# software-mansion/smelter

Measured on NVIDIA H100. Metric: 4K composited frames/sec (16-input grid) per GPU, higher is better.
Workload: dtype f32 math on u8 planes (f16 resampler scratch)

## Files before the change

include/smelter_b200.h:

```cpp
#ifndef SMELTER_B200_H
#define SMELTER_B200_H

#include <stddef.h>
#include <stdint.h>

#ifdef __cplusplus
extern "C" {
#endif

typedef struct smr_renderer smr_renderer;

typedef enum {
    SMR_OK = 0,
    SMR_ERR_INVALID_ARGUMENT = 1,
    SMR_ERR_CUDA = 2,
    SMR_ERR_OUTPUT_NOT_REGISTERED = 3,
    SMR_ERR_SCENE = 4,
    SMR_ERR_UNSUPPORTED = 5,
    SMR_ERR_OUT_OF_MEMORY = 6,
    SMR_ERR_BUFFER_TOO_SMALL = 7
} smr_status;

typedef enum { SMR_MODE_GPU_OPTIMIZED = 0, SMR_MODE_CPU_OPTIMIZED = 1 } smr_rendering_mode;

// ... 254 lines not shown
    uint32_t n_glyphs;
    const smr_atlas *mask_atlas, *color_atlas;
    int32_t color_mode;
} smr_text;

smr_status smr_debug_partition(const int32_t *dst_w, const int32_t *dst_h, uint32_t n_jobs, uint32_t max_blocks,
                               int32_t *pieces, uint32_t pieces_cap, uint32_t *n_pieces, int32_t *begin,
                               uint32_t begin_cap, uint32_t *n_blocks);

smr_status smr_debug_weights(float scale, float offset, uint32_t n_out, float *weights, size_t cap, uint32_t *taps, float *inv,
                             int32_t *first);
smr_status smr_debug_sincos(const float *x, uint32_t n, float *s, float *c);

smr_status smr_debug_tile_plan(const int32_t *boxes, uint32_t n_layers, uint32_t width, uint32_t height, int32_t sorted,
                               int32_t *owner_layer, uint32_t owner_cap, uint32_t *tiles, uint32_t tiles_cap, uint32_t *n_tiles);

typedef enum {
    SMR_FUSED_LDG = 0,
    SMR_FUSED_TMA_INT = 1,
    SMR_FUSED_TMA_ANY = 2
} smr_fused_kernel;
typedef struct {
    int32_t kernel;
    int32_t ratio;
    int32_t window;
    int32_t box;
    int32_t src_class;
    int32_t full_range;
    int32_t v_same;
    int32_t strip_cols;
// ... 103 lines not shown
```

smelter_b200/_ffi.py:

```python
import ctypes as C
import os

_HERE = os.path.dirname(os.path.abspath(__file__))
LIB_PATH = os.environ.get("SMR_LIB_PATH") or os.path.join(_HERE, "libsmelter_b200.so")

SMR_OK = 0
STATUS_NAMES = {0: "SMR_OK", 1: "SMR_ERR_INVALID_ARGUMENT", 2: "SMR_ERR_CUDA", 3: "SMR_ERR_OUTPUT_NOT_REGISTERED",
                4: "SMR_ERR_SCENE", 5: "SMR_ERR_UNSUPPORTED", 6: "SMR_ERR_OUT_OF_MEMORY", 7: "SMR_ERR_BUFFER_TOO_SMALL"}

MODE_GPU_OPTIMIZED, MODE_CPU_OPTIMIZED = 0, 1
COMPONENT_INPUT_STREAM, COMPONENT_VIEW, COMPONENT_TILES, COMPONENT_RESCALER = 0, 1, 2, 3
COMPONENT_SHADER, COMPONENT_WEB_VIEW, COMPONENT_IMAGE, COMPONENT_TEXT = 4, 5, 6, 7
FRAME_PLANAR_YUV420, FRAME_PLANAR_YUVJ420, FRAME_NV12, FRAME_BGRA, FRAME_ARGB, FRAME_RGBA8 = 0, 1, 2, 3, 4, 5
FRAME_PLANAR_YUV422, FRAME_PLANAR_YUV444, FRAME_UYVY422, FRAME_YUYV422 = 6, 7, 8, 9
MEM_HOST, MEM_DEVICE = 0, 1
WEB_CHROMIUM_EMBEDDING, WEB_NATIVE_OVER_CONTENT, WEB_NATIVE_UNDER_CONTENT = 0, 1, 2
OUT_PLANAR_YUV420, OUT_PLANAR_YUV422, OUT_PLANAR_YUV444, OUT_RGBA8, OUT_NV12 = 0, 1, 2, 3, 4
MAX_MASKS = 20


class Options(C.Structure):
    _fields_ = [("cuda_device", C.c_int32), ("rendering_mode", C.c_int32), ("max_layouts_count", C.c_uint32),
                ("stream_fallback_timeout_ns", C.c_uint64), ("framerate_num", C.c_uint32), ("framerate_den", C.c_uint32)]

# ... 175 lines not shown
                ("tex_pitch", C.c_int32 * 3), ("tex_align", C.c_int32 * 3), ("width", C.c_int32), ("height", C.c_int32),
                ("out_format", C.c_int32)]


KERNEL_CLASSES = ["convert", "weights", "resample_box", "resample_first", "resample_last", "composite", "output",
                  "fill", "resample_fused", "image", "web", "shader"]


class KernelTimes(C.Structure):
    _fields_ = [("total_ms", C.c_double * len(KERNEL_CLASSES)), ("launches", C.c_uint64 * len(KERNEL_CLASSES))]


EXPORTS = [
    "smr_create", "smr_destroy", "smr_register_input", "smr_unregister_input", "smr_register_image", "smr_unregister_image",
    "smr_register_web_renderer", "smr_unregister_web_renderer", "smr_web_set_frame", "smr_web_set_child_rects", "smr_register_shader", "smr_unregister_shader", "smr_register_wgsl_shader", "smr_update_scene",
    "smr_unregister_output", "smr_set_layouts", "smr_render", "smr_render_begin", "smr_render_end", "smr_preprocess_frame", "smr_premultiply_rgba8", "smr_render_text", "smr_debug_partition", "smr_debug_tile_plan", "smr_debug_weights", "smr_debug_sincos", "smr_debug_fused_jobs", "smr_debug_resample_stages", "smr_debug_composite_layers", "smr_debug_interior", "smr_output_plane_sizes",
    "smr_component_default", "smr_debug_layouts", "smr_debug_node_layouts", "smr_debug_image_nodes", "smr_debug_set_inputs", "smr_get_stats", "smr_set_profiling", "smr_get_kernel_times",
    "smr_comm_get_unique_id", "smr_comm_init", "smr_comm_broadcast_inputs", "smr_comm_exchange_inputs", "smr_comm_pull_inputs", "smr_peer_pool_alloc", "smr_peer_pool_open", "smr_peer_pool_close", "smr_peer_pool_free", "smr_comm_destroy", "smr_host_register", "smr_host_unregister", "smr_cuda_stream", "smr_last_error",
    "smr_version",
]

_lib = None


def lib():
    global _lib
    if _lib is not None:
        return _lib
    if not os.path.exists(LIB_PATH):
        raise ImportError(
            f"{LIB_PATH} is missing: build it with `python -m smelter_b200.build` "
# ... 20 lines not shown
        f.argtypes = [vp, C.c_uint64, C.POINTER(InputFrame), C.c_uint32, C.POINTER(OutputFrame), C.c_uint32]
    L.smr_render_end.argtypes = [vp]
    L.smr_preprocess_frame.argtypes = [vp, C.POINTER(InputFrame), C.c_uint32, C.c_uint32, C.c_void_p, C.c_uint32, C.c_int32]
    L.smr_preprocess_frame.restype = C.c_int32
    L.smr_premultiply_rgba8.argtypes = [vp, C.POINTER(InputFrame), C.c_void_p, C.c_uint32, C.c_int32]
    L.smr_premultiply_rgba8.restype = C.c_int32
    L.smr_render_text.argtypes = [vp, C.c_uint32, C.c_uint32, Rgba, C.c_void_p, C.c_uint32, C.POINTER(Atlas), C.POINTER(Atlas),
                                  C.c_int32, C.c_void_p, C.c_uint32, C.c_int32]
    L.smr_render_text.restype = C.c_int32
    L.smr_debug_partition.argtypes = [C.POINTER(C.c_int32), C.POINTER(C.c_int32), C.c_uint32, C.c_uint32, C.POINTER(C.c_int32),
                                      C.c_uint32, C.POINTER(C.c_uint32), C.POINTER(C.c_int32), C.c_uint32, C.POINTER(C.c_uint32)]
    L.smr_debug_partition.restype = C.c_int32
    L.smr_debug_tile_plan.argtypes = [C.POINTER(C.c_int32), C.c_uint32, C.c_uint32, C.c_uint32, C.c_int32, C.POINTER(C.c_int32), C.c_uint32,
                                      C.POINTER(C.c_uint32), C.c_uint32, C.POINTER(C.c_uint32)]
    L.smr_debug_tile_plan.restype = C.c_int32
    L.smr_debug_weights.argtypes = [C.c_float, C.c_float, C.c_uint32, C.c_void_p, C.c_size_t, C.POINTER(C.c_uint32), C.c_void_p,
                                    C.c_void_p]
    L.smr_debug_weights.restype = C.c_int32
    L.smr_debug_sincos.argtypes = [C.c_void_p, C.c_uint32, C.c_void_p, C.c_void_p]
    L.smr_debug_sincos.restype = C.c_int32
    L.smr_debug_fused_jobs.argtypes = [vp, C.POINTER(FusedJobInfo), C.c_uint32, C.POINTER(C.c_uint32)]
    L.smr_debug_fused_jobs.restype = C.c_int32
    L.smr_debug_resample_stages.argtypes = [vp, C.POINTER(ResampleStageInfo), C.c_uint32, C.POINTER(C.c_uint32),
                                            C.POINTER(C.c_int32), C.c_uint32, C.POINTER(C.c_uint32)]
    L.smr_debug_resample_stages.restype = C.c_int32
    L.smr_debug_composite_layers.argtypes = [vp, C.POINTER(CompositeLayerInfo), C.c_uint32, C.POINTER(C.c_uint32)]
    L.smr_debug_composite_layers.restype = C.c_int32
    L.smr_debug_interior.argtypes = [C.POINTER(RenderLayout), C.c_uint32, C.c_uint32, C.POINTER(C.c_int32 * 12), C.c_void_p]
    L.smr_debug_interior.restype = C.c_int32
    L.smr_output_plane_sizes.argtypes = [C.c_uint32, C.c_uint32, C.c_int32, C.POINTER(C.c_size_t * 3)]
# ... 35 lines not shown
```

smelter_b200/csrc/kernels.cu:

```cuda
#include <cuda_fp16.h>
#include <cuda_runtime.h>

#include <cstdio>
#include <cstdlib>
#include <atomic>
#include <cstring>

#include "kernels.h"
#include "interior.h"
#include "int_weights.h"

namespace smr {
namespace dev {

#include "ptx_helpers.cuh"

#define ENC_KEY0 ((127 - 13) << 5)
#define ENC_KEYS ((13 << 5) + 1)
__device__ unsigned char c_enc0[420];

#include "node_sample.cuh"

static thread_local char g_err[256] = {0};
const char *last_launch_error() { return g_err; }
// ... 880 lines not shown
#define PARAM_LAYERS kCompositeParamLayers
#define MAX_LUT 4
struct CompositeParams {
    CompositeJob job;
    LayerDev layers[PARAM_LAYERS];
};

template <bool PARAM>
__device__ __forceinline__ void composite_body(const CompositeJob &J, const LayerDev *__restrict__ LAYERS) {
    __shared__ Tables T;
    __shared__ unsigned short s_list[MAX_TILE_LAYERS];
    __shared__ int s_count;
    __shared__ LayerDev s_layers[PARAM ? 1 : SM_LAYERS];
    static_assert(CB_X * CT_W == kDirectTileW && CB_Y * CT_H * CT_ITERS == kDirectTileH, "direct tiles are the block tiles");
    int tile_x = blockIdx.x, tile_y = blockIdx.y;
    if (J.tile_list != nullptr) {
        if ((int)blockIdx.x >= J.n_tiles || blockIdx.y != 0) return;
        const uint32_t t = __ldg(J.tile_list + blockIdx.x);
        tile_x = (int)(t & 0xffffu); tile_y = (int)(t >> 16);
    } else if (J.direct_map != nullptr && __ldg(J.direct_map + tile_y * J.map_w + tile_x)) return;
    load_tables(T);
    const int tile_x0 = tile_x * (CB_X * CT_W), tile_y0 = tile_y * (CB_Y * CT_H * CT_ITERS);
    const int tile_x1 = min(tile_x0 + CB_X * CT_W, J.width), tile_y1 = min(tile_y0 + CB_Y * CT_H * CT_ITERS, J.height);
    {
        __shared__ int s_wc[CB_Y];
        const int tid = threadIdx.y * CB_X + threadIdx.x;
        int base_count = 0;
        for (int base = 0; base < J.n_layers; base += CB_X * CB_Y) {
            const int i = base + tid;
            bool hit = false;
            if (i < J.n_layers) {
                int4 bb;
                if (PARAM) bb = make_int4(LAYERS[i].px0, LAYERS[i].px1, LAYERS[i].py0, LAYERS[i].py1);
                else bb = __ldg(reinterpret_cast<const int4 *>(&LAYERS[i].px0));
                hit = bb.x < tile_x1 && bb.y > tile_x0 && bb.z < tile_y1 && bb.w > tile_y0;
            }
            const unsigned m = __ballot_sync(0xffffffffu, hit);
            if (threadIdx.x == 0) s_wc[threadIdx.y] = __popc(m);
            __syncthreads();
// ... 11 lines not shown
    }
    __syncthreads();
    if (!PARAM) {
        const int nsm = min(s_count, SM_LAYERS);
        const int words = (int)(sizeof(LayerDev) / 4);
        const int tid = threadIdx.y * CB_X + threadIdx.x;
        for (int i = tid; i < nsm * words; i += CB_X * CB_Y) {
            int l = i / words, w = i - l * words;
            reinterpret_cast<unsigned int *>(&s_layers[l])[w] =
                __ldg(reinterpret_cast<const unsigned int *>(&LAYERS[s_list[l]]) + w);
        }
    }
    __syncthreads();

    __shared__ uchar4 s_lut[MAX_LUT][CB_X * CB_Y];
    __shared__ uchar4 s_px[CB_Y][CB_X * CT_W * CT_H];
    __shared__ unsigned char s_items[CB_Y][CB_X * CT_W * CT_H];
    static_assert(CB_X == 32 && CB_X * CT_W * CT_H <= 256, "one warp per tile row, items fit a byte");
    static_assert(CB_X * CB_Y == 256, "one table entry per thread");
    {
        const int tid = threadIdx.y * CB_X + threadIdx.x;
        int nl = 0;
        for (int li = 0; li < s_count && nl < MAX_LUT; li++) {
            const LayerDev &L = PARAM ? LAYERS[s_list[li]] : (li < SM_LAYERS ? s_layers[li] : LAYERS[s_list[li]]);
            if (L.fast & FAST_LUT) {
                s_lut[nl][tid] = blend(T, J.mode, make_uchar4(tid, tid, tid, tid),
                                       make_float4(L.color[0], L.color[1], L.color[2], L.color[3]));
                nl++;
            }
        }
        if (nl) __syncthreads();
    }

// ... 176 lines not shown
                            px[j][i] = blend(T, J.mode, px[j][i], make_float4(lut[t.x], lut[t.y], lut[t.z], T.u8n[t.w]));
                        }
                    }
                break;
            }
            general = true;
        } while (0);
        unsigned need = 0;
        if (general) {
#pragma unroll 1
            for (int k = 0; k < CT_W * CT_H; k++) {
                const int X = x0 + (k & (CT_W - 1)), Y = y0 + k / CT_W;
                if (X < J.width && Y < J.height && quad_covers(L, X, Y)) need |= 1u << k;
            }
        }
        if (__ballot_sync(0xffffffffu, need != 0) == 0) continue;
        const int lane = threadIdx.x;
        const int cnt = __popc(need);
        int incl = cnt;
#pragma unroll
        for (int d = 1; d < 32; d <<= 1) {
            const int t = __shfl_up_sync(0xffffffffu, incl, d);
            if (lane >= d) incl += t;
        }
        const int total = __shfl_sync(0xffffffffu, incl, 31);
        if (total > 5 * 32) {
            for (int k = 0; k < CT_W * CT_H; k++) {
                if (!((need >> k) & 1u)) continue;
                const int i = k & (CT_W - 1), j = k / CT_W;
                uchar4 cur = j == 0 ? (i == 0 ? px[0][0] : i == 1 ? px[0][1] : i == 2 ? px[0][2] : px[0][3])
                                    : (i == 0 ? px[1][0] : i == 1 ? px[1][1] : i == 2 ? px[1][2] : px[1][3]);
                uchar4 res = shade_blend(T, J, L, x0 + i, y0 + j, cur);
#pragma unroll
                for (int jj = 0; jj < CT_H; jj++)
#pragma unroll
                    for (int ii = 0; ii < CT_W; ii++)
                        if (jj == j && ii == i) px[jj][ii] = res;
            }
            continue;
        }
        unsigned char *items = s_items[threadIdx.y];
        uchar4 *spx = s_px[threadIdx.y];
        if (need) {
            int o = incl - cnt;
#pragma unroll
            for (int k = 0; k < CT_W * CT_H; k++) {
                spx[lane * (CT_W * CT_H) + k] = px[k / CT_W][k & (CT_W - 1)];
                if ((need >> k) & 1u) items[o++] = (unsigned char)(lane * (CT_W * CT_H) + k);
            }
        }
        __syncwarp();
        for (int base = 0; base < total; base += 32) {
            const int idx = base + lane;
            if (idx < total) {
                const int item = items[idx], k = item & (CT_W * CT_H - 1);
                const int X = tile_x0 + (item / (CT_W * CT_H)) * CT_W + (k & (CT_W - 1)), Y = y0 + k / CT_W;
                spx[item] = shade_blend(T, J, L, X, Y, spx[item]);
            }
        }
        __syncwarp();
        if (need) {
#pragma unroll
            for (int k = 0; k < CT_W * CT_H; k++) px[k / CT_W][k & (CT_W - 1)] = spx[lane * (CT_W * CT_H) + k];
        }
    }

    if (x0 >= J.width || y0 >= J.height) continue;
    if (J.out_format < 0 || J.out_format == 3) {
        const bool vec16 = (((uintptr_t)J.out0 | (uintptr_t)J.out_pitch0) & 15) == 0;
#pragma unroll
        for (int j = 0; j < CT_H; j++) {
            int Y = y0 + j;
            if (Y >= J.height) break;
            uchar4 *row = reinterpret_cast<uchar4 *>(J.out0 + (size_t)Y * J.out_pitch0);
            if (x0 + CT_W <= J.width && vec16) {
                uint4 v;
                v.x = *reinterpret_cast<unsigned int *>(&px[j][0]);
                v.y = *reinterpret_cast<unsigned int *>(&px[j][1]);
// ... 335 lines not shown
```

smelter_b200/csrc/kernels.h:

```cpp
#pragma once

#include <cstddef>
#include <cstdint>

namespace smr {
namespace dev {

enum TexKind : int32_t {
    TEX_NONE = 0,
    TEX_RGBA8 = 1,
    TEX_YUV420 = 2,
    TEX_NV12 = 3,
    TEX_F16 = 4,
    TEX_BGRA = 5,
    TEX_ARGB = 6,
    TEX_YUV422 = 7,
    TEX_YUV444 = 8,
    TEX_UYVY = 9,
    TEX_YUYV = 10,
};
inline
#ifdef __CUDACC__
__host__ __device__
#endif
// ... 42 lines not shown

struct CompositeJob {
    int32_t width, height;
    int32_t mode;
    int32_t n_layers;
    const LayerDev *layers;
    const uint32_t *tile_list;
    const MaskDev *masks;
    const Tex *textures;
    int32_t out_format;
    uint8_t *out0, *out1, *out2;
    int32_t out_pitch0, out_pitch1, out_pitch2;
    const uint8_t *direct_map;
    int32_t map_w;
    int32_t n_tiles;
};
constexpr int kDirectTileW = 128, kDirectTileH = 16;
constexpr int kCompositeParamLayers = 96;

constexpr uint64_t kMaxBoxTexels = 1ull << 24;

struct ResampleJob {
    Tex src;
    int32_t axis;
    int32_t perp_offset;
    int32_t taps;
    int32_t dst_w, dst_h;
    int32_t dst_f16;
    uint8_t *dst;
    int32_t dst_pitch;
// ... 149 lines not shown
```

smelter_b200/csrc/node_sample.cuh:

```cuda

__device__ float c_u8n[256];
__device__ float c_dec[256];
__device__ float c_thr[256];
__device__ float c_yl[256];
#define ENC1_KEY0 ((127 - 13) << 8)
#define ENC1_KEYS ((13 << 8) + 1)
__device__ unsigned char c_enc1[ENC1_KEYS + 3];

struct Tables {
    float u8n[256];
    float dec[256];
    float thr[256];
    float yl[256];
};

__device__ __forceinline__ void load_tables(Tables &t) {
    for (int i = threadIdx.y * blockDim.x + threadIdx.x; i < 256; i += blockDim.x * blockDim.y) {
        t.u8n[i] = c_u8n[i];
        t.dec[i] = c_dec[i];
        t.thr[i] = c_thr[i];
        t.yl[i] = c_yl[i];
    }
    __syncthreads();
}

__device__ __forceinline__ float clamp01(float x) { return __saturatef(x); }

__device__ __forceinline__ int unorm8(float x) { return __float2int_rn(clamp01(x) * 255.0f); }

__device__ __forceinline__ int srgb_encode(const Tables &t, float lin) {
    const float x = clamp01(lin);
    const int k = max((__float_as_int(x) >> 15) - ENC1_KEY0, 0);
    const int e = __ldg(c_enc1 + k);
    return e + (x >= t.thr[e] ? 1 : 0);
}

struct LinTap {
// ... 285 lines not shown
```

smelter_b200/csrc/renderer.cpp:

```cpp
#include <cuda.h>
#include <cuda_runtime.h>
#include <dlfcn.h>

#include <algorithm>
#include <array>
#include <cmath>
#include <cstdio>
#include <cstring>
#include <deque>
#include <map>
#include <memory>
#include <mutex>
#include <string>
#include <tuple>
#include <vector>

#include "../../include/smelter_b200.h"
#include "interior.h"
#include "kernels.h"
#include "scene.h"
#include "wgsl.h"

namespace smr {

// ... 395 lines not shown
    struct Output {
        OutputNode node;
        std::vector<std::unique_ptr<TextNode>> texts;
        std::vector<std::unique_ptr<ImageNode>> images;
        std::vector<std::unique_ptr<WebNode>> webs;
        std::vector<std::unique_ptr<ShaderNode>> shaders;
        std::deque<Input> nested;
        uint64_t nodes_planned = 0;
        int32_t format = 0;
        Resolution res;
        DevBuf planes[kTicksInFlight][3];
        uint64_t tile_key = 0;
        bool tile_key_valid = false;
        std::vector<int> tile_owner_layer;
        std::vector<uint32_t> tile_list;
    };
    struct WeightKey {
        uint32_t scale_bits, offset_bits;
        int32_t n_out;
        bool operator<(const WeightKey &o) const {
            return std::tie(scale_bits, offset_bits, n_out) < std::tie(o.scale_bits, o.offset_bits, o.n_out);
        }
    };
    struct WeightEntry {
        float *weights = nullptr, *inv = nullptr;
        int32_t *first = nullptr;
        int taps = 0;
        uint64_t last_used = 0;
    };

// ... 85 lines not shown
    };
    struct StageRec {
        dev::ResampleJob job;
        int src_tex;
        size_t src_off, dst_off;
    };
    struct OutputRec { dev::OutputJob job; int src_tex; };
    struct CompositeRec {
        dev::CompositeJob job; size_t layers_off, masks_off;
        size_t out_frame_off = SIZE_MAX;
        size_t direct_off = SIZE_MAX;
        std::vector<int> direct_owner;
        bool use_list = false;
        std::vector<uint32_t> list;
        size_t list_off = SIZE_MAX;
    };
    struct PendingCopy { void *dst; size_t dpitch; const void *src; size_t spitch; size_t width, height; };
    struct Fill { uint8_t *p[3]; int pitch[3]; int w, h, fmt; uint8_t yuv[3]; };
    struct TickPlan {
        std::vector<TexRec> tex;
        std::vector<StageRec> stages[3];
        std::vector<FusedRec> fused;
        std::vector<CUtensorMap> tmaps;
        std::vector<dev::WeightJob> weight_jobs;
        std::vector<std::pair<int, size_t>> convert_jobs;
        std::vector<CompositeRec> composites;
        std::vector<OutputRec> outputs;
        std::vector<Fill> fills;
        std::vector<PendingCopy> d2h;
        std::vector<TextNode *> texts;
// ... 17 lines not shown
    smr_status make_image_node(const ImageParams &p, std::unique_ptr<ImageNode> &out);
    smr_status make_web_node(const WebParams &p, std::unique_ptr<WebNode> &out);
    void plan_web_node(Output &o, WebNode &n);
    smr_status make_shader_node(const ShaderParams &p, std::unique_ptr<ShaderNode> &out);
    void plan_shader_node(Output &o, ShaderNode &n, uint64_t pts);
    std::vector<std::pair<void *, cudaEvent_t>> retired_shaders_;
    void reap_shaders(bool all);
    cudaEvent_t web_ev_ = nullptr;
    cudaMemPool_t web_pool_ = nullptr;
    smr_status alloc_on_stream(size_t bytes, std::shared_ptr<void> &buf);
    Output &install_output(const char *output_id, OutputNode &&node, int32_t fmt, uint32_t w, uint32_t h);
    void plan_node_textures(Output &o, uint64_t pts);
    CompositeRec composite_rec(int W, int H, const std::vector<dev::LayerDev> &layers, const std::vector<dev::MaskDev> &masks);
    int composite_texture(CompositeRec pc);
    void plan_tiles(Output &o, CompositeRec &pc, const std::vector<dev::LayerDev> &layers, int W, int H);
    std::vector<WeightKey> new_weight_keys_;
    void rollback_weights();
    struct TmapKey {
        uintptr_t p; int pitch, w, h, kind;
        bool operator<(const TmapKey &o) const { return std::tie(p, pitch, w, h, kind) < std::tie(o.p, o.pitch, o.w, o.h, o.kind); }
    };
    std::map<TmapKey, CUtensorMap> tmap_cache_;
    std::map<std::tuple<uint32_t, uint32_t, int32_t, int32_t>, uint8_t *> lane_perms_;
    const uint8_t *lane_perm(float scale, float offset, int n_out, int cols);
    bool plane_tmap(const uint8_t *p, int pitch, int w, int h, int kind, CUtensorMap *out);
    bool direct_k11_ = true;

    std::vector<uint8_t> param_host_;
    size_t param_used_ = 0;
    PinnedBuf param_pinned_[kTicksInFlight];
    DevBuf param_dev_[kTicksInFlight];
    size_t frame_used_ = 0;
    DevBuf frame_dev_;
    std::map<WeightKey, WeightEntry> weights_;
    cudaStream_t copy_stream_ = nullptr, copy_stream2_ = nullptr;
    cudaStream_t d2h_stream_ = nullptr;
    cudaEvent_t kernels_done_[kTicksInFlight] = {};
    cudaEvent_t h2d_done2_[kTicksInFlight] = {};
    int upload_rr_ = 0;
    cudaEvent_t h2d_done_[kTicksInFlight] = {}, tick_done_[kTicksInFlight] = {};
    cudaStream_t comm_stream_ = nullptr;
// ... 73 lines not shown
    }
}

static double eotf_f64(double c) { return c <= 0.04045 ? c / 12.92 : std::pow((c + 0.055) / 1.055, 2.4); }
static const std::array<float, 255> kSrgbEncodeThr = [] {
    std::array<float, 255> thr;
    for (int k = 0; k < 255; k++) thr[k] = (float)eotf_f64(((double)k + 0.5) / 255.0);
    return thr;
}();

smr_status Renderer::init() {
    if (opts_.max_layouts_count == 0) opts_.max_layouts_count = 100;
    if (opts_.max_layouts_count > 1024) opts_.max_layouts_count = 1024;
    if (opts_.cuda_device == -1) { host_only_ = true; return SMR_OK; }
    if (const char *e = getenv("SMR_DIRECT_K11")) direct_k11_ = e[0] != '0';
    int n = 0;
    cudaError_t e = cudaGetDeviceCount(&n);
    if (e != cudaSuccess || n <= 0) {
        set_error("no CUDA device: the H100 compositor has no CPU fallback");
        return SMR_ERR_CUDA;
    }
    if (opts_.cuda_device < 0 || opts_.cuda_device >= n) {
        set_error("cuda_device out of range");
        return SMR_ERR_INVALID_ARGUMENT;
    }
    int cc_major = 0, cc_minor = 0;
    CUDA_OK(cudaDeviceGetAttribute(&cc_major, cudaDevAttrComputeCapabilityMajor, opts_.cuda_device));
    CUDA_OK(cudaDeviceGetAttribute(&cc_minor, cudaDevAttrComputeCapabilityMinor, opts_.cuda_device));
    if (cc_major != 9 || cc_minor != 0) {
        set_error("device has compute capability " + std::to_string(cc_major) + "." + std::to_string(cc_minor) +
// ... 1169 lines not shown
static void out_plane_layout(int fmt, uint32_t w, uint32_t h, size_t row_bytes[3], size_t rows[3]) {
    for (int i = 0; i < 3; i++) row_bytes[i] = rows[i] = 0;
    int icw, ich;
    dev::chroma_dims(fmt, (int)w, (int)h, icw, ich);
    uint32_t cw = (uint32_t)icw, ch = (uint32_t)ich;
    if (fmt == SMR_OUT_RGBA8) { row_bytes[0] = (size_t)w * 4; rows[0] = h; }
    else if (fmt == SMR_OUT_NV12) { row_bytes[0] = w; rows[0] = h; row_bytes[1] = (size_t)cw * 2; rows[1] = ch; }
    else { row_bytes[0] = w; rows[0] = h; row_bytes[1] = row_bytes[2] = cw; rows[1] = rows[2] = ch; }
}

static inline void fnv1a(uint64_t &h, const void *p, size_t n) {
    const uint8_t *b = (const uint8_t *)p;
    for (size_t i = 0; i < n; i++) { h ^= b[i]; h *= 1099511628211ull; }
}
struct TileLayerBox { int32_t px0, px1, py0, py1, ix0, ix1, iy0, iy1, jx0, jx1, jy0, jy1, opaque, job; };
void plan_tiles_core(const TileLayerBox *boxes, int n_layers, int W, int H, bool sort, std::vector<int> &owner_layer,
                     std::vector<uint32_t> &list) {
    const int TW = dev::kDirectTileW, TH = dev::kDirectTileH;
    const int tx_n = (W + TW - 1) / TW, ty_n = (H + TH - 1) / TH;
    const size_t n_tiles = (size_t)tx_n * ty_n;
    owner_layer.assign(n_tiles, -1);
    std::vector<std::pair<int, uint32_t>> keyed;
    keyed.reserve(n_tiles);
    std::map<int, int> layer_of_job;
    for (int ty = 0; ty < ty_n; ty++)
        for (int tx = 0; tx < tx_n; tx++) {
            const int x0 = tx * TW, y0 = ty * TH, x1 = std::min(x0 + TW, W), y1 = std::min(y0 + TH, H);
            int cost = 0;
            bool top = true;
            int owner = -1;
// ... 43 lines not shown
            job_of[li] = ji;
        }
    uint64_t key = 1469598103934665603ull;
    fnv1a(key, &W, sizeof(W)); fnv1a(key, &H, sizeof(H));
    if (!layers.empty()) fnv1a(key, layers.data(), sizeof(dev::LayerDev) * layers.size());
    if (!job_of.empty()) fnv1a(key, job_of.data(), sizeof(int) * job_of.size());
    const size_t n_tiles = (size_t)tx_n * ty_n;
    if (!(o.tile_key_valid && o.tile_key == key && o.tile_owner_layer.size() == n_tiles)) {
        std::vector<TileLayerBox> boxes(layers.size());
        for (size_t li = 0; li < layers.size(); li++) {
            const dev::LayerDev &L = layers[li];
            boxes[li] = {L.px0, L.px1, L.py0, L.py1, L.ix0, L.ix1, L.iy0, L.iy1, L.jx0, L.jx1, L.jy0, L.jy1,
                         (L.fast & dev::FAST_OPAQUE) ? 1 : 0, job_of[li]};
        }
        plan_tiles_core(boxes.data(), (int)boxes.size(), W, H, true, o.tile_owner_layer, o.tile_list);
        o.tile_key = key; o.tile_key_valid = true;
    }
    pc.use_list = true;
    pc.list = o.tile_list;
    pc.job.map_w = tx_n;
    std::map<int, int> claimed;
    bool any = false;
    pc.direct_owner.assign(n_tiles, -1);
    for (size_t t = 0; t < n_tiles; t++) {
        const int li = o.tile_owner_layer[t];
        if (li < 0) continue;
        pc.direct_owner[t] = job_of[li];
        claimed[job_of[li]] = li;
        any = true;
    }
    if (!any) { pc.direct_owner.clear(); return; }
    pc.direct_off = param_alloc(n_tiles);
    for (auto &jl : claimed) {
        dev::FusedJob &fj = plan_.fused[jl.first].job;
        const dev::LayerDev &L = layers[jl.second];
        plan_.fused[jl.first].direct_off = pc.direct_off;
        fj.map_w = tx_n;
        fj.direct_id = jl.first + 1;
        fj.fx = -L.tx_off; fj.fy = -L.ty_off;
        fj.out_format = cj.out_format;
        fj.out0 = cj.out0; fj.out1 = cj.out1; fj.out2 = cj.out2;
        fj.out_pitch0 = cj.out_pitch0; fj.out_pitch1 = cj.out_pitch1; fj.out_pitch2 = cj.out_pitch2;
    }
}

Renderer::LayoutEval Renderer::eval_layout(Output &o, LayoutParams &lp, uint64_t pts) {
    LayoutEval e;
    for (const NodeRef &r : lp.children) {
        Input *in = node_input(o, r);
        e.child_in.push_back(in);
        e.child_res.push_back(in ? std::optional<Resolution>(in->res) : std::nullopt);
    }
    e.res = lp.resolution(pts);
    e.layouts = lp.layouts(pts, e.child_res);
    return e;
}

Renderer::Input *Renderer::node_input(Output &o, const NodeRef &r) {
// ... 385 lines not shown
                idx.push_back((int)ji); widths.push_back(f.job.dst_w); heights.push_back(f.job.dst_h); cols.push_back(shape.strip_cols);
            }
            std::vector<dev::FusedPiece> pieces;
            std::vector<int> begin;
            partition_fused_rows(idx.data(), widths.data(), heights.data(), (int)idx.size(), sm_count_ * shape.groups_per_sm, pieces,
                                 begin, dev::kFusedStripCols, cols.data(), shape.row_gran);
            if (pieces.empty()) continue;
            for (const dev::FusedPiece &pp : pieces)
                if (plan_.fused[pp.job].direct_off != SIZE_MAX && ((pp.oy_begin | pp.oy_end) & 1)) {
                    plan_.fused[pp.job].direct_off = SIZE_MAX;
                    for (CompositeRec &pc : plan_.composites)
                        for (size_t t = 0; t < pc.direct_owner.size(); t++)
                            if (pc.direct_owner[t] == pp.job) {
                                pc.direct_owner[t] = -1;
                                pc.list.push_back((uint32_t)(t % (size_t)pc.job.map_w) | ((uint32_t)(t / (size_t)pc.job.map_w) << 16));
                            }
                }
            fused_launches.push_back({v, param_put(pieces.data(), sizeof(dev::FusedPiece) * pieces.size()),
                                      param_put(begin.data(), sizeof(int) * begin.size()), (int)begin.size() - 1});
        }
    }
    const size_t tex_off = param_put_all(plan_.tex, &TexRec::tex);
    size_t stage_off[3];
    for (int s = 0; s < 3; s++) stage_off[s] = param_put_all(plan_.stages[s], &StageRec::job);
    const size_t wj_off = param_put(plan_.weight_jobs.data(), sizeof(dev::WeightJob) * plan_.weight_jobs.size());
    const size_t tm_off = param_put(plan_.tmaps.data(), sizeof(CUtensorMap) * plan_.tmaps.size());
    uint64_t direct_tiles = 0;
    for (CompositeRec &pc : plan_.composites) {
        if (pc.direct_off != SIZE_MAX) {
            bool any = false;
            for (size_t t = 0; t < pc.direct_owner.size(); t++) {
                param_host_[pc.direct_off + t] = pc.direct_owner[t] >= 0 ? (uint8_t)(pc.direct_owner[t] + 1) : 0;
                any = any || pc.direct_owner[t] >= 0;
                direct_tiles += pc.direct_owner[t] >= 0 ? 1 : 0;
            }
            if (!any) pc.direct_off = SIZE_MAX;
        }
        if (pc.use_list) {
            pc.list_off = param_put(pc.list.data(), sizeof(uint32_t) * pc.list.size());
            pc.job.n_tiles = (int)pc.list.size();
        }
    }
    const size_t fj_off = param_put_all(plan_.fused, &FusedRec::job);
    const size_t cj_off = param_put_all(plan_.composites, &CompositeRec::job);
    const TileJobs text_jobs = param_put_tile_jobs(plan_.texts, &TextNode::job);
    const TileJobs image_jobs = param_put_tile_jobs(plan_.images, &ImageNode::job);
    std::vector<std::vector<WebNode *>> web_launches;
    std::vector<TileJobs> web_jobs;
    {
        for (WebNode *n : plan_.webs) {
            for (size_t i = 0; i < n->planes.size(); i++)
                if (n->plane_child[i] >= 0) n->planes[i].tex = packed_node_tex(*n->owner, n->params.children[n->plane_child[i]]);
            n->planes_off = param_put(n->planes.data(), sizeof(dev::WebPlane) * n->planes.size());
        }
        std::vector<WebNode *> order = plan_.webs;
// ... 44 lines not shown
        const FusedRec &f = plan_.fused[i];
        if (f.tmap_idx >= 0) {
            const uint8_t *m = pd + tm_off + sizeof(CUtensorMap) * (size_t)f.tmap_idx;
            fj[i].tm0 = m; fj[i].tm1 = m + sizeof(CUtensorMap); fj[i].tm2 = m + 2 * sizeof(CUtensorMap);
        }
        fj[i].direct_map = dev_ptr(f.direct_off);
    }
    dev::CompositeJob *cj = reinterpret_cast<dev::CompositeJob *>(param_host_.data() + cj_off);
    for (size_t i = 0; i < plan_.composites.size(); i++) {
        const CompositeRec &c = plan_.composites[i];
        cj[i].layers = (const dev::LayerDev *)(pd + c.layers_off);
        cj[i].masks = (const dev::MaskDev *)(pd + c.masks_off);
        cj[i].textures = (const dev::Tex *)(pd + tex_off);
        cj[i].direct_map = dev_ptr(c.direct_off);
        cj[i].tile_list = (const uint32_t *)dev_ptr(c.list_off);
    }
    memcpy(param_pinned_[slot_].p, param_host_.data(), param_used_);
    CUDA_OK(cudaMemcpyAsync(pd, param_pinned_[slot_].p, param_used_, cudaMemcpyHostToDevice, stream_));

    auto launched = [&](int n) -> bool { if (n < 0) return false; launches += (uint64_t)n; return true; };
    auto launch_webs = [&](int depth) -> bool {
        for (size_t l = 0; l < web_launches.size(); l++) {
            if (web_launches[l][0]->params.depth != depth) continue;
            const TileJobs &t = web_jobs[l];
            if (!launched(dev::launch_web((const dev::WebJob *)(pd + t.jobs_off), (const int32_t *)(pd + t.begin_off),
                                          (int)web_launches[l].size(), t.n_tiles, stream_))) return false;
            prof_mark(SMR_KERNEL_WEB);
        }
        return true;
    };
// ... 727 lines not shown
        std::vector<int> owner;
        std::vector<uint32_t> list;
        smr::plan_tiles_core(reinterpret_cast<const smr::TileLayerBox *>(boxes), (int)n_layers, (int)width, (int)height, sorted != 0, owner, list);
        *n_tiles = (uint32_t)list.size();
        if (owner_layer) {
            if (owner_cap < owner.size()) return SMR_ERR_BUFFER_TOO_SMALL;
            for (size_t i = 0; i < owner.size(); i++) owner_layer[i] = owner[i];
        }
        if (tiles) {
            if (tiles_cap < list.size()) return SMR_ERR_BUFFER_TOO_SMALL;
            memcpy(tiles, list.data(), sizeof(uint32_t) * list.size());
        }
        return SMR_OK;
    } catch (...) { return SMR_ERR_OUT_OF_MEMORY; }
}
smr_status smr_output_plane_sizes(uint32_t w, uint32_t h, int32_t fmt, size_t sizes[3]) {
    if (!sizes) return SMR_ERR_INVALID_ARGUMENT;
    if (fmt < SMR_OUT_PLANAR_YUV420 || fmt > SMR_OUT_NV12) return SMR_ERR_UNSUPPORTED;
    size_t rb[3], rows[3];
    smr::out_plane_layout(fmt, w, h, rb, rows);
    for (int i = 0; i < 3; i++) sizes[i] = rb[i] * rows[i];
    return SMR_OK;
}

void smr_component_default(int32_t type, smr_component *c) {
    if (!c) return;
    memset(c, 0, sizeof(*c));
    c->type = type;
    c->direction = SMR_DIRECTION_ROW;
    c->overflow = SMR_OVERFLOW_HIDDEN;
// ... 9 lines not shown
```

Baseline: 1853.

## Precompute per-tile layer lists on host and compact shading work block-wide

The host now builds a per-tile list of overlapping layers for list-driven composite tiles, so the kernel loads it directly instead of culling all layers per block. The per-warp compaction of pixels needing shading becomes a block-wide compaction with shared counts, so all 256 threads share the shade_blend work. It also adds a debug env var to restrict tiles by class, plus a debug FFI export. This costs more host planning, a larger parameter upload and extra block-wide __syncthreads per layer, and it drops the fast path for heavy warps.

Result: no change. 1858, median of 6 (+0.3%).

```diff
diff --git a/include/smelter_b200.h b/include/smelter_b200.h
--- a/include/smelter_b200.h
+++ b/include/smelter_b200.h
@@ -292,6 +292,8 @@
 
 smr_status smr_debug_tile_plan(const int32_t *boxes, uint32_t n_layers, uint32_t width, uint32_t height, int32_t sorted,
                                int32_t *owner_layer, uint32_t owner_cap, uint32_t *tiles, uint32_t tiles_cap, uint32_t *n_tiles);
+smr_status smr_debug_tile_layers(const int32_t *boxes, uint32_t n_layers, uint32_t width, uint32_t height, uint32_t *begin,
+                                 uint32_t begin_cap, uint16_t *layers, uint32_t layers_cap, uint32_t *n_tiles, uint32_t *n_entries);
 
 typedef enum {
     SMR_FUSED_LDG = 0,
diff --git a/smelter_b200/_ffi.py b/smelter_b200/_ffi.py
--- a/smelter_b200/_ffi.py
+++ b/smelter_b200/_ffi.py
@@ -213,7 +213,7 @@
 EXPORTS = [
     "smr_create", "smr_destroy", "smr_register_input", "smr_unregister_input", "smr_register_image", "smr_unregister_image",
     "smr_register_web_renderer", "smr_unregister_web_renderer", "smr_web_set_frame", "smr_web_set_child_rects", "smr_register_shader", "smr_unregister_shader", "smr_register_wgsl_shader", "smr_update_scene",
-    "smr_unregister_output", "smr_set_layouts", "smr_render", "smr_render_begin", "smr_render_end", "smr_preprocess_frame", "smr_premultiply_rgba8", "smr_render_text", "smr_debug_partition", "smr_debug_tile_plan", "smr_debug_weights", "smr_debug_sincos", "smr_debug_fused_jobs", "smr_debug_resample_stages", "smr_debug_composite_layers", "smr_debug_interior", "smr_output_plane_sizes",
+    "smr_unregister_output", "smr_set_layouts", "smr_render", "smr_render_begin", "smr_render_end", "smr_preprocess_frame", "smr_premultiply_rgba8", "smr_render_text", "smr_debug_partition", "smr_debug_tile_plan", "smr_debug_tile_layers", "smr_debug_weights", "smr_debug_sincos", "smr_debug_fused_jobs", "smr_debug_resample_stages", "smr_debug_composite_layers", "smr_debug_interior", "smr_output_plane_sizes",
     "smr_component_default", "smr_debug_layouts", "smr_debug_node_layouts", "smr_debug_image_nodes", "smr_debug_set_inputs", "smr_get_stats", "smr_set_profiling", "smr_get_kernel_times",
     "smr_comm_get_unique_id", "smr_comm_init", "smr_comm_broadcast_inputs", "smr_comm_exchange_inputs", "smr_comm_pull_inputs", "smr_peer_pool_alloc", "smr_peer_pool_open", "smr_peer_pool_close", "smr_peer_pool_free", "smr_comm_destroy", "smr_host_register", "smr_host_unregister", "smr_cuda_stream", "smr_last_error",
     "smr_version",
@@ -264,6 +264,9 @@
     L.smr_debug_tile_plan.argtypes = [C.POINTER(C.c_int32), C.c_uint32, C.c_uint32, C.c_uint32, C.c_int32, C.POINTER(C.c_int32), C.c_uint32,
                                       C.POINTER(C.c_uint32), C.c_uint32, C.POINTER(C.c_uint32)]
     L.smr_debug_tile_plan.restype = C.c_int32
+    L.smr_debug_tile_layers.argtypes = [C.POINTER(C.c_int32), C.c_uint32, C.c_uint32, C.c_uint32, C.POINTER(C.c_uint32), C.c_uint32,
+                                        C.POINTER(C.c_uint16), C.c_uint32, C.POINTER(C.c_uint32), C.POINTER(C.c_uint32)]
+    L.smr_debug_tile_layers.restype = C.c_int32
     L.smr_debug_weights.argtypes = [C.c_float, C.c_float, C.c_uint32, C.c_void_p, C.c_size_t, C.POINTER(C.c_uint32), C.c_void_p,
                                     C.c_void_p]
     L.smr_debug_weights.restype = C.c_int32
diff --git a/smelter_b200/csrc/kernels.cu b/smelter_b200/csrc/kernels.cu
--- a/smelter_b200/csrc/kernels.cu
+++ b/smelter_b200/csrc/kernels.cu
@@ -918,15 +918,23 @@
     __shared__ LayerDev s_layers[PARAM ? 1 : SM_LAYERS];
     static_assert(CB_X * CT_W == kDirectTileW && CB_Y * CT_H * CT_ITERS == kDirectTileH, "direct tiles are the block tiles");
     int tile_x = blockIdx.x, tile_y = blockIdx.y;
+    uint32_t list_begin = 0, list_end = 0;
     if (J.tile_list != nullptr) {
         if ((int)blockIdx.x >= J.n_tiles || blockIdx.y != 0) return;
         const uint32_t t = __ldg(J.tile_list + blockIdx.x);
         tile_x = (int)(t & 0xffffu); tile_y = (int)(t >> 16);
+        list_begin = __ldg(J.tile_layer_begin + blockIdx.x);
+        list_end = __ldg(J.tile_layer_begin + blockIdx.x + 1);
     } else if (J.direct_map != nullptr && __ldg(J.direct_map + tile_y * J.map_w + tile_x)) return;
-    load_tables(T);
+    load_tables_nosync(T);
     const int tile_x0 = tile_x * (CB_X * CT_W), tile_y0 = tile_y * (CB_Y * CT_H * CT_ITERS);
     const int tile_x1 = min(tile_x0 + CB_X * CT_W, J.width), tile_y1 = min(tile_y0 + CB_Y * CT_H * CT_ITERS, J.height);
-    {
+    if (J.tile_list != nullptr) {
+        const int tid = threadIdx.y * CB_X + threadIdx.x;
+        const int cnt = min((int)(list_end - list_begin), MAX_TILE_LAYERS);
+        for (int i = tid; i < cnt; i += CB_X * CB_Y) s_list[i] = __ldg(J.tile_layers + list_begin + i);
+        if (tid == 0) s_count = cnt;
+    } else {
         __shared__ int s_wc[CB_Y];
         const int tid = threadIdx.y * CB_X + threadIdx.x;
         int base_count = 0;
@@ -968,9 +976,10 @@
     __syncthreads();
 
     __shared__ uchar4 s_lut[MAX_LUT][CB_X * CB_Y];
-    __shared__ uchar4 s_px[CB_Y][CB_X * CT_W * CT_H];
-    __shared__ unsigned char s_items[CB_Y][CB_X * CT_W * CT_H];
-    static_assert(CB_X == 32 && CB_X * CT_W * CT_H <= 256, "one warp per tile row, items fit a byte");
+    __shared__ uchar4 s_px[CB_X * CB_Y * CT_W * CT_H];
+    __shared__ unsigned short s_items[CB_X * CB_Y * CT_W * CT_H];
+    __shared__ int s_need[2][CB_Y];
+    static_assert(CB_X == 32 && CT_W * CT_H == 8, "one warp per tile row, a thread's pixels are item bits 0..2");
     static_assert(CB_X * CB_Y == 256, "one table entry per thread");
     {
         const int tid = threadIdx.y * CB_X + threadIdx.x;
@@ -1177,8 +1186,7 @@
                 if (X < J.width && Y < J.height && quad_covers(L, X, Y)) need |= 1u << k;
             }
         }
-        if (__ballot_sync(0xffffffffu, need != 0) == 0) continue;
-        const int lane = threadIdx.x;
+        const int lane = threadIdx.x, tid = threadIdx.y * CB_X + threadIdx.x;
         const int cnt = __popc(need);
         int incl = cnt;
 #pragma unroll
@@ -1186,45 +1194,35 @@
             const int t = __shfl_up_sync(0xffffffffu, incl, d);
             if (lane >= d) incl += t;
         }
-        const int total = __shfl_sync(0xffffffffu, incl, 31);
-        if (total > 5 * 32) {
+        if (lane == 31) s_need[li & 1][threadIdx.y] = incl;
+        __syncthreads();
+        int total = 0, before = 0;
+#pragma unroll
+        for (int w = 0; w < CB_Y; w++) {
+            const int c = s_need[li & 1][w];
+            total += c;
+            before += w < (int)threadIdx.y ? c : 0;
+        }
+        if (total == 0) continue;
+        if (need) {
+            int o = before + incl - cnt;
+#pragma unroll
             for (int k = 0; k < CT_W * CT_H; k++) {
-                if (!((need >> k) & 1u)) continue;
-                const int i = k & (CT_W - 1), j = k / CT_W;
-                uchar4 cur = j == 0 ? (i == 0 ? px[0][0] : i == 1 ? px[0][1] : i == 2 ? px[0][2] : px[0][3])
-                                    : (i == 0 ? px[1][0] : i == 1 ? px[1][1] : i == 2 ? px[1][2] : px[1][3]);
-                uchar4 res = shade_blend(T, J, L, x0 + i, y0 + j, cur);
-#pragma unroll
-                for (int jj = 0; jj < CT_H; jj++)
-#pragma unroll
-                    for (int ii = 0; ii < CT_W; ii++)
-                        if (jj == j && ii == i) px[jj][ii] = res;
-            }
-            continue;
-        }
-        unsigned char *items = s_items[threadIdx.y];
-        uchar4 *spx = s_px[threadIdx.y];
+                s_px[tid * (CT_W * CT_H) + k] = px[k / CT_W][k & (CT_W - 1)];
+                if ((need >> k) & 1u) s_items[o++] = (unsigned short)(tid * (CT_W * CT_H) + k);
+            }
+        }
+        __syncthreads();
+        for (int idx = tid; idx < total; idx += CB_X * CB_Y) {
+            const int item = s_items[idx], t = item / (CT_W * CT_H), k = item & (CT_W * CT_H - 1);
+            const int X = tile_x0 + (t % CB_X) * CT_W + (k & (CT_W - 1));
+            const int Y = tile_y0 + (it * CB_Y + t / CB_X) * CT_H + k / CT_W;
+            s_px[item] = shade_blend(T, J, L, X, Y, s_px[item]);
+        }
+        __syncthreads();
         if (need) {
-            int o = incl - cnt;
-#pragma unroll
-            for (int k = 0; k < CT_W * CT_H; k++) {
-                spx[lane * (CT_W * CT_H) + k] = px[k / CT_W][k & (CT_W - 1)];
-                if ((need >> k) & 1u) items[o++] = (unsigned char)(lane * (CT_W * CT_H) + k);
-            }
-        }
-        __syncwarp();
-        for (int base = 0; base < total; base += 32) {
-            const int idx = base + lane;
-            if (idx < total) {
-                const int item = items[idx], k = item & (CT_W * CT_H - 1);
-                const int X = tile_x0 + (item / (CT_W * CT_H)) * CT_W + (k & (CT_W - 1)), Y = y0 + k / CT_W;
-                spx[item] = shade_blend(T, J, L, X, Y, spx[item]);
-            }
-        }
-        __syncwarp();
-        if (need) {
-#pragma unroll
-            for (int k = 0; k < CT_W * CT_H; k++) px[k / CT_W][k & (CT_W - 1)] = spx[lane * (CT_W * CT_H) + k];
+#pragma unroll
+            for (int k = 0; k < CT_W * CT_H; k++) px[k / CT_W][k & (CT_W - 1)] = s_px[tid * (CT_W * CT_H) + k];
         }
     }
 
diff --git a/smelter_b200/csrc/kernels.h b/smelter_b200/csrc/kernels.h
--- a/smelter_b200/csrc/kernels.h
+++ b/smelter_b200/csrc/kernels.h
@@ -80,6 +80,8 @@
     const uint8_t *direct_map;
     int32_t map_w;
     int32_t n_tiles;
+    const uint32_t *tile_layer_begin;
+    const uint16_t *tile_layers;
 };
 constexpr int kDirectTileW = 128, kDirectTileH = 16;
 constexpr int kCompositeParamLayers = 96;
diff --git a/smelter_b200/csrc/node_sample.cuh b/smelter_b200/csrc/node_sample.cuh
--- a/smelter_b200/csrc/node_sample.cuh
+++ b/smelter_b200/csrc/node_sample.cuh
@@ -14,13 +14,16 @@
     float yl[256];
 };
 
-__device__ __forceinline__ void load_tables(Tables &t) {
+__device__ __forceinline__ void load_tables_nosync(Tables &t) {
     for (int i = threadIdx.y * blockDim.x + threadIdx.x; i < 256; i += blockDim.x * blockDim.y) {
         t.u8n[i] = c_u8n[i];
         t.dec[i] = c_dec[i];
         t.thr[i] = c_thr[i];
         t.yl[i] = c_yl[i];
     }
+}
+__device__ __forceinline__ void load_tables(Tables &t) {
+    load_tables_nosync(t);
     __syncthreads();
 }
 
diff --git a/smelter_b200/csrc/renderer.cpp b/smelter_b200/csrc/renderer.cpp
--- a/smelter_b200/csrc/renderer.cpp
+++ b/smelter_b200/csrc/renderer.cpp
@@ -433,6 +433,8 @@
         bool tile_key_valid = false;
         std::vector<int> tile_owner_layer;
         std::vector<uint32_t> tile_list;
+        std::vector<uint32_t> tile_layer_begin;
+        std::vector<uint16_t> tile_layers;
     };
     struct WeightKey {
         uint32_t scale_bits, offset_bits;
@@ -548,6 +550,9 @@
         bool use_list = false;
         std::vector<uint32_t> list;
         size_t list_off = SIZE_MAX;
+        std::vector<uint32_t> layer_begin;
+        std::vector<uint16_t> layer_idx;
+        size_t layer_begin_off = SIZE_MAX, layer_idx_off = SIZE_MAX;
     };
     struct PendingCopy { void *dst; size_t dpitch; const void *src; size_t spitch; size_t width, height; };
     struct Fill { uint8_t *p[3]; int pitch[3]; int w, h, fmt; uint8_t yuv[3]; };
@@ -595,6 +600,7 @@
     CompositeRec composite_rec(int W, int H, const std::vector<dev::LayerDev> &layers, const std::vector<dev::MaskDev> &masks);
     int composite_texture(CompositeRec pc);
     void plan_tiles(Output &o, CompositeRec &pc, const std::vector<dev::LayerDev> &layers, int W, int H);
+    void debug_restrict_tiles(CompositeRec &pc, const std::vector<dev::LayerDev> &layers) const;
     std::vector<WeightKey> new_weight_keys_;
     void rollback_weights();
     struct TmapKey {
@@ -606,6 +612,7 @@
     const uint8_t *lane_perm(float scale, float offset, int n_out, int cols);
     bool plane_tmap(const uint8_t *p, int pitch, int w, int h, int kind, CUtensorMap *out);
     bool direct_k11_ = true;
+    int debug_tile_class_ = -1;
 
     std::vector<uint8_t> param_host_;
     size_t param_used_ = 0;
@@ -709,6 +716,11 @@
     if (opts_.max_layouts_count > 1024) opts_.max_layouts_count = 1024;
     if (opts_.cuda_device == -1) { host_only_ = true; return SMR_OK; }
     if (const char *e = getenv("SMR_DIRECT_K11")) direct_k11_ = e[0] != '0';
+    if (const char *e = getenv("SMR_DEBUG_TILE_CLASS")) {
+        static const char *names[] = {"split", "corner", "overlay", "edge", "empty"};
+        for (int i = 0; i < 5; i++)
+            if (strcmp(e, names[i]) == 0) debug_tile_class_ = i;
+    }
     int n = 0;
     cudaError_t e = cudaGetDeviceCount(&n);
     if (e != cudaSuccess || n <= 0) {
@@ -1908,6 +1920,23 @@
     for (size_t i = 0; i < n; i++) { h ^= b[i]; h *= 1099511628211ull; }
 }
 struct TileLayerBox { int32_t px0, px1, py0, py1, ix0, ix1, iy0, iy1, jx0, jx1, jy0, jy1, opaque, job; };
+template <class B>
+static void append_tile_layers(const B *ls, int n_layers, int W, int H, uint32_t t, std::vector<uint16_t> &idx) {
+    const int x0 = (int)(t & 0xffffu) * dev::kDirectTileW, y0 = (int)(t >> 16) * dev::kDirectTileH;
+    const int x1 = std::min(x0 + dev::kDirectTileW, W), y1 = std::min(y0 + dev::kDirectTileH, H);
+    for (int li = 0; li < n_layers; li++)
+        if (ls[li].px0 < x1 && ls[li].px1 > x0 && ls[li].py0 < y1 && ls[li].py1 > y0) idx.push_back((uint16_t)li);
+}
+template <class B>
+static void tile_layer_lists(const B *ls, int n_layers, int W, int H, const std::vector<uint32_t> &list,
+                             std::vector<uint32_t> &begin, std::vector<uint16_t> &idx) {
+    begin.assign(1, 0);
+    idx.clear();
+    for (uint32_t t : list) {
+        append_tile_layers(ls, n_layers, W, H, t, idx);
+        begin.push_back((uint32_t)idx.size());
+    }
+}
 void plan_tiles_core(const TileLayerBox *boxes, int n_layers, int W, int H, bool sort, std::vector<int> &owner_layer,
                      std::vector<uint32_t> &list) {
     const int TW = dev::kDirectTileW, TH = dev::kDirectTileH;
@@ -1981,10 +2010,14 @@
                          (L.fast & dev::FAST_OPAQUE) ? 1 : 0, job_of[li]};
         }
         plan_tiles_core(boxes.data(), (int)boxes.size(), W, H, true, o.tile_owner_layer, o.tile_list);
+        tile_layer_lists(boxes.data(), (int)boxes.size(), W, H, o.tile_list, o.tile_layer_begin, o.tile_layers);
         o.tile_key = key; o.tile_key_valid = true;
     }
     pc.use_list = true;
     pc.list = o.tile_list;
+    pc.layer_begin = o.tile_layer_begin;
+    pc.layer_idx = o.tile_layers;
+    if (debug_tile_class_ >= 0) debug_restrict_tiles(pc, layers);
     pc.job.map_w = tx_n;
     std::map<int, int> claimed;
     bool any = false;
@@ -2009,6 +2042,37 @@
         fj.out0 = cj.out0; fj.out1 = cj.out1; fj.out2 = cj.out2;
         fj.out_pitch0 = cj.out_pitch0; fj.out_pitch1 = cj.out_pitch1; fj.out_pitch2 = cj.out_pitch2;
     }
+}
+
+void Renderer::debug_restrict_tiles(CompositeRec &pc, const std::vector<dev::LayerDev> &layers) const {
+    if (debug_tile_class_ == 4) { pc.job.n_layers = 0; std::fill(pc.layer_begin.begin(), pc.layer_begin.end(), 0u); pc.layer_idx.clear(); return; }
+    std::vector<uint32_t> list, begin(1, 0);
+    std::vector<uint16_t> idx;
+    for (size_t k = 0; k < pc.list.size(); k++) {
+        const uint32_t t = pc.list[k];
+        const float x0 = (float)((t & 0xffffu) * dev::kDirectTileW), y0 = (float)((t >> 16) * dev::kDirectTileH);
+        const float x1 = x0 + dev::kDirectTileW, y1 = y0 + dev::kDirectTileH;
+        bool overlay = false, corner = false;
+        int textures = 0;
+        for (uint32_t i = pc.layer_begin[k]; i < pc.layer_begin[k + 1]; i++) {
+            const dev::LayerDev &L = layers[pc.layer_idx[i]];
+            overlay |= (L.fast & dev::FAST_LUT) != 0;
+            textures += L.type == 0;
+            const float r = std::max(std::max(L.border_radius[0], L.border_radius[1]), std::max(L.border_radius[2], L.border_radius[3]));
+            if (r > 0.0f && std::isfinite(L.int_corner)) {
+                const float c = L.int_corner, l = L.left, tp = L.top, rt = L.left + L.content_w, bt = L.top + L.content_h;
+                const bool cx = (x0 < l + c && x1 > l) || (x0 < rt && x1 > rt - c);
+                const bool cy = (y0 < tp + c && y1 > tp) || (y0 < bt && y1 > bt - c);
+                corner |= cx && cy;
+            }
+        }
+        const int cls = overlay ? 2 : corner ? 1 : textures >= 2 ? 0 : 3;
+        if (cls != debug_tile_class_) continue;
+        list.push_back(t);
+        idx.insert(idx.end(), pc.layer_idx.begin() + pc.layer_begin[k], pc.layer_idx.begin() + pc.layer_begin[k + 1]);
+        begin.push_back((uint32_t)idx.size());
+    }
+    pc.list.swap(list); pc.layer_begin.swap(begin); pc.layer_idx.swap(idx);
 }
 
 Renderer::LayoutEval Renderer::eval_layout(Output &o, LayoutParams &lp, uint64_t pts) {
@@ -2424,6 +2488,9 @@
                             if (pc.direct_owner[t] == pp.job) {
                                 pc.direct_owner[t] = -1;
                                 pc.list.push_back((uint32_t)(t % (size_t)pc.job.map_w) | ((uint32_t)(t / (size_t)pc.job.map_w) << 16));
+                                append_tile_layers(reinterpret_cast<const dev::LayerDev *>(param_host_.data() + pc.layers_off),
+                                                   pc.job.n_layers, pc.job.width, pc.job.height, pc.list.back(), pc.layer_idx);
+                                pc.layer_begin.push_back((uint32_t)pc.layer_idx.size());
                             }
                 }
             fused_launches.push_back({v, param_put(pieces.data(), sizeof(dev::FusedPiece) * pieces.size()),
@@ -2449,6 +2516,8 @@
         if (pc.use_list) {
             pc.list_off = param_put(pc.list.data(), sizeof(uint32_t) * pc.list.size());
             pc.job.n_tiles = (int)pc.list.size();
+            pc.layer_begin_off = param_put(pc.layer_begin.data(), sizeof(uint32_t) * pc.layer_begin.size());
+            pc.layer_idx_off = param_put(pc.layer_idx.data(), sizeof(uint16_t) * pc.layer_idx.size());
         }
     }
     const size_t fj_off = param_put_all(plan_.fused, &FusedRec::job);
@@ -2523,6 +2592,8 @@
         cj[i].textures = (const dev::Tex *)(pd + tex_off);
         cj[i].direct_map = dev_ptr(c.direct_off);
         cj[i].tile_list = (const uint32_t *)dev_ptr(c.list_off);
+        cj[i].tile_layer_begin = (const uint32_t *)dev_ptr(c.layer_begin_off);
+        cj[i].tile_layers = (const uint16_t *)dev_ptr(c.layer_idx_off);
     }
     memcpy(param_pinned_[slot_].p, param_host_.data(), param_used_);
     CUDA_OK(cudaMemcpyAsync(pd, param_pinned_[slot_].p, param_used_, cudaMemcpyHostToDevice, stream_));
@@ -3280,6 +3351,31 @@
         return SMR_OK;
     } catch (...) { return SMR_ERR_OUT_OF_MEMORY; }
 }
+smr_status smr_debug_tile_layers(const int32_t *boxes, uint32_t n_layers, uint32_t width, uint32_t height, uint32_t *begin,
+                                 uint32_t begin_cap, uint16_t *layers, uint32_t layers_cap, uint32_t *n_tiles, uint32_t *n_entries) {
+    if ((n_layers && !boxes) || n_layers > 65536 || !n_tiles || !n_entries || width == 0 || height == 0 || width > 16384 * 4 ||
+        height > 16384 * 4)
+        return SMR_ERR_INVALID_ARGUMENT;
+    try {
+        const smr::TileLayerBox *b = reinterpret_cast<const smr::TileLayerBox *>(boxes);
+        std::vector<int> owner;
+        std::vector<uint32_t> list, bg;
+        std::vector<uint16_t> idx;
+        smr::plan_tiles_core(b, (int)n_layers, (int)width, (int)height, true, owner, list);
+        smr::tile_layer_lists(b, (int)n_layers, (int)width, (int)height, list, bg, idx);
+        *n_tiles = (uint32_t)list.size();
+        *n_entries = (uint32_t)idx.size();
+        if (begin) {
+            if (begin_cap < bg.size()) return SMR_ERR_BUFFER_TOO_SMALL;
+            memcpy(begin, bg.data(), sizeof(uint32_t) * bg.size());
+        }
+        if (layers) {
+            if (layers_cap < idx.size()) return SMR_ERR_BUFFER_TOO_SMALL;
+            memcpy(layers, idx.data(), sizeof(uint16_t) * idx.size());
+        }
+        return SMR_OK;
+    } catch (...) { return SMR_ERR_OUT_OF_MEMORY; }
+}
 smr_status smr_output_plane_sizes(uint32_t w, uint32_t h, int32_t fmt, size_t sizes[3]) {
     if (!sizes) return SMR_ERR_INVALID_ARGUMENT;
     if (fmt < SMR_OUT_PLANAR_YUV420 || fmt > SMR_OUT_NV12) return SMR_ERR_UNSUPPORTED;
```
